# CLSFramework/gym-soccer-2d-env

Hardware: AMD Instinct MI355X
Metric: env-steps/sec at 65536 parallel reach_ball envs per MI355X (higher is better)
Workload: dtype f32

## Files before the change

gym-soccer-2d-env_amd/csrc/s2d_engine.hip:

```cpp
#include <hip/hip_runtime.h>

#include <cmath>
#include <cstdio>
#include <cstdlib>
#include <cstring>
#include <new>
#include <string>
#include <type_traits>

#include "s2d_device.h"

#include "s2d_actor_launch.h"
#include "s2d_kernels.h"

__global__ void s2d_tables_kernel(S2DHot p, const S2DRare* __restrict__ rp, S2DTables* __restrict__ t) {
  if (blockIdx.x == 0 && threadIdx.x == 0 && rp->tab_len > 0) tables_build(p, rp->recover_init, rp->tab_power, rp->tab_len, *t);
}
__global__ __launch_bounds__(kBlock) void s2d_init_kernel(S2DHot p, const S2DRare* __restrict__ rp,
                                                          float* __restrict__ S, int64_t stride, int64_t n) {
  int64_t i = (int64_t)blockIdx.x * kBlock + threadIdx.x;
  if (i >= n) return;
  S[F_STAMINA * stride + i] = p.stamina_max;
  S[F_RECOVERY * stride + i] = rp->recover_init;
  S[F_EFFORT * stride + i] = p.effort_init;
// ... 264 lines not shown
      sc_lut[k] = make_float2(sn, cs);
    }
    __syncthreads();
  }
  if (wave_first >= n) return;
  const bool active = i < n;
  int64_t rows = n - wave_first; if (rows > kWave) rows = kWave;
  const int valid = (int)rows * S2D_OBS_DIM;
  const bool use_k = uses_policy_step<MODE, NOISE>(kind);
  uint32_t* const kplane = reinterpret_cast<uint32_t*>(S + F_POLICY * stride);
  Env e;
  uint32_t gl = 0, gh = 0, k0 = 0;
  if (active) {
    env_load(e, S, stride, i);
    if (use_k) k0 = kplane[i];
    uint64_t gid = (((uint64_t)p.gid_hi << 32) | p.gid_lo) + (uint64_t)i;
    gl = (uint32_t)gid; gh = (uint32_t)(gid >> 32);
    asm volatile("" ::"v"(e.px), "v"(e.py), "v"(e.vx), "v"(e.vy), "v"(e.body), "v"(e.stamina), "v"(e.effort),
                 "v"(e.recovery), "v"(e.capacity), "v"(e.bx), "v"(e.by), "v"(e.bvx), "v"(e.bvy), "v"(e.prev_dist),
                 "v"(e.prev_angle), "v"(e.step_number), "v"(e.cycle), "v"(k0));
  }
  bool fast = false;
  if (tab_len > 0) {
    bool ok = true;
    if (active) {
      const int sn = e.step_number;
      ok = sn >= 0 && sn < tab_len;
      const int q = ok ? sn : 0;
      ok = ok && e.stamina == tb->stamina[q] && e.effort == tb->effort[q] && e.recovery == tb->recovery[q] &&
           e.capacity == tb->capacity[q] && e.body == rintf(e.body) && fabsf(e.body) <= 180.0f;
    }
    fast = __ballot(active && !ok) == 0ull;
  }
  ObsOut ob;
  float reward = 0.0f, dir = 0.0f; int done = 0, res = 0, cmd = 0;
  unsigned int cnt1 = 0, cnt2 = 0, cnt3 = 0;
  float* const term_row = o.terminal_obs + i * S2D_OBS_DIM;
  U4 quad{0, 0, 0, 0}, squad{0, 0, 0, 0};
  bool have_prep = false;
  uint32_t* const coop_scratch = reinterpret_cast<uint32_t*>(&lds[wv][0]);
  if (p.auto_reset) {
    prep_fill_coop<NK>(p, rp, prep[wv], lane, active ? reset_key(e) : 0u, gl, gh, active, coop_scratch);
    have_prep = active;
  }
  int n_missing = 0;
  int64_t row = 0;
  const bool lut = NOISE && MODE == S2D_MODE_DISCRETE && kind == S2D_ACT_RANDOM && p.n_actions <= kWave;
  if (lut && lane < p.n_actions) {
    int c0; float pw, d0;
    action_map<MODE>(p, Action4{(float)lane, 0.0f, 0.0f, 0.0f}, 0.0f, c0, pw, d0);
    const CmdPrep c = cmd_prepare(p, c0, pw, d0);
    act_lut[wv][lane] = make_float4(c.power, c.dir, c.dir_rate, d0);
  }
  for (int t = 0; t < n_steps; ++t, row += n) {
    res = 0;
    if (n_missing >= kRefillMin) {
      if (active && !have_prep) { prep_fill<NK>(p, rp, prep[wv], lane, e, gl, gh); have_prep = true; }
      n_missing = 0;
    }
    if (active) {
      const uint32_t k = k0 + (uint32_t)t;
      CmdPrep c;
      if (lut) {
        if (t == 0 || (k & 3u) == 0u) quad = policy_quad(p, gl, gh, k, S2D_ST_POLICY);
        const int a = (int)rnd_below(quad_word(quad, k), (uint32_t)p.n_actions);
        if (ro.action) static_cast<int32_t*>(ro.action)[row + i] = a;
        const float4 e4 = act_lut[wv][a];
        c = CmdPrep{e4.x, e4.y, e4.z}; dir = e4.w; cmd = S2D_CMD_DASH;
      } else {
        c = decide<MODE>(p, actions, kind, row + i, gl, gh, k, t == 0 || (k & 3u) == 0u, quad, squad, ro.action, cmd, dir);
      }
      if (fast) step_env<NK, true>(p, rp, e, gl, gh, k, cmd, c, ob, reward, done, res, term_row, &prep[wv], lane, have_prep, ep_lds, sc_lut);
      else step_env<NK, false>(p, rp, e, gl, gh, k, cmd, c, ob, reward, done, res, term_row, &prep[wv], lane, have_prep);
      if (ro.reward) ro.reward[row + i] = reward;
      if (ro.done) ro.done[row + i] = (uint8_t)done;
      if (ro.result) ro.result[row + i] = (uint8_t)res;
      cnt1 += res == S2D_RESULT_GOAL; cnt2 += res == S2D_RESULT_OUT; cnt3 += res == S2D_RESULT_TIMEOUT;
    }
    if (p.auto_reset) n_missing += __popcll(__ballot(active && done != 0));
    if (ro.obs) store_obs_tile(lds[wv], ob, lane, active, ro.obs + (row + wave_first) * S2D_OBS_DIM, valid);
  }
  if (active) {
    if (fast) {
      const int q = e.step_number;
      e.stamina = tb->stamina[q]; e.effort = tb->effort[q]; e.recovery = tb->recovery[q]; e.capacity = tb->capacity[q];
    }
    env_store(e, S, stride, i);
    if (use_k) kplane[i] = k0 + (uint32_t)n_steps;
    o.reward[i] = reward; o.done[i] = (uint8_t)done; o.result[i] = (uint8_t)res;
    o.action_dir[i] = dir; o.action_cmd[i] = (uint8_t)cmd;
  }
  store_obs_tile(lds[wv], ob, lane, active, o.obs + wave_first * S2D_OBS_DIM, valid);
  if (!active) { cnt1 = cnt2 = cnt3 = 0; }
#pragma unroll
  for (int off = 32; off > 0; off >>= 1) {
    cnt1 += __shfl_xor(cnt1, off); cnt2 += __shfl_xor(cnt2, off); cnt3 += __shfl_xor(cnt3, off);
  }
  unsigned long long* const srow = stats_row(o.stats, wave_first);
  stats_store(srow, lane, stats_load(srow, lane), wave_first == 0 ? (unsigned long long)n * (unsigned long long)n_steps : 0ull, cnt1, cnt2, cnt3);
}

#ifndef S2D_NPRIO_S
#define S2D_NPRIO_S 3
#endif
#ifndef S2D_NPRIO_A
#define S2D_NPRIO_A 2
#endif
#ifndef S2D_NPRIO_B
#define S2D_NPRIO_B 2
#endif
#ifndef S2D_NPRIO_P
#define S2D_NPRIO_P 1
#endif
#ifndef S2D_PRIO_S
#define S2D_PRIO_S 1
#endif
#ifndef S2D_PRIO_A
#define S2D_PRIO_A 2
#endif
#ifndef S2D_PRIO_B
#define S2D_PRIO_B 3
#endif

#ifdef S2D_STAMPS
#define WS_STAMP_DECL uint64_t st_busy = 0, st_t0 = __builtin_amdgcn_s_memtime(); const uint64_t st_begin = st_t0, st_rt0 = __builtin_amdgcn_s_memrealtime()
#define WS_BARRIER() do { st_busy += __builtin_amdgcn_s_memtime() - st_t0; __syncthreads(); st_t0 = __builtin_amdgcn_s_memtime(); } while (0)
#define WS_STAMP_STORE() do { if (lane == 0) { float* q_ = o.terminal_obs + (wave_first + 2 * role) * S2D_OBS_DIM; \
    q_[0] = (float)st_busy; q_[1] = (float)(__builtin_amdgcn_s_memtime() - st_begin); q_[2] = (float)(st_rt0 & 0xffffff); \
    q_[3] = (float)(__builtin_amdgcn_s_memrealtime() & 0xffffff); \
    q_[4] = __int_as_float((int)__builtin_amdgcn_s_getreg((31 << 11) | 4)); q_[5] = __int_as_float((int)__builtin_amdgcn_s_getreg((31 << 11) | 20)); } } while (0)
#else
#define WS_STAMP_DECL do {} while (0)
#define WS_BARRIER() __syncthreads()
#define WS_STAMP_STORE() do {} while (0)
#endif

template <int MODE, int NK, int REC = 0>
__global__ __launch_bounds__(kWsBlock, 4) void s2d_reach_rollout_ws_kernel(S2DHot p_sgpr, const S2DRare* __restrict__ rp,
                                                                        float* __restrict__ S, int64_t stride,
                                                                        int64_t n, int n_steps,
                                                                        const void* __restrict__ actions, int kind,
                                                                        RolloutOut ro, StepOut o) {
  constexpr bool NOISE = NK != S2D_NK_OFF;
  constexpr int kActWords = NOISE ? (int)WA_WORDS : (int)WA_NPM;
  __shared__ float act[3][kActWords][kWave];
  __shared__ float snap[2][WS_WORDS][kWave];
  __shared__ float slots[kSlots][SL_WORDS][kWave];
  __shared__ __attribute__((aligned(16))) float tile[2][kObsTile];
  __shared__ float4 act_lut[kWave];
  __shared__ float ep_lds[S2D_TAB_MAX];
  __shared__ float2 sc_lut[361];
  const int lane = threadIdx.x & (kWave - 1);
  const int role = __builtin_amdgcn_readfirstlane(threadIdx.x / kWave);
  const bool nt = REC == 2 || (REC == 0 && ro.nt != 0);
  const int64_t wave_first = (int64_t)blockIdx.x * kWave;
  const int64_t i = wave_first + lane;
  const bool active = i < n;
  int64_t rows = n - wave_first; rows = rows > kWave ? kWave : rows;
  const int valid = (int)rows * S2D_OBS_DIM;
  const int n_iter = n_steps + 3;

  if (role != 1 && p_sgpr.auto_reset) {
    const uint64_t gid = (((uint64_t)p_sgpr.gid_hi << 32) | p_sgpr.gid_lo) + (uint64_t)i;
    uint32_t ep0 = 0u;
    if (active) ep0 = reinterpret_cast<const uint32_t*>(S + F_EPISODE * stride)[i];
    const int k = role == 0 ? 0 : role - 1;
    slot_fill_coop<NK>(p_sgpr, rp, slots[k], lane, (uint32_t)gid, (uint32_t)(gid >> 32), ep0 + 1u + (uint32_t)k, active,
                          reinterpret_cast<uint32_t*>(&tile[0][0]) + role * kWave);
  }

  if (role == 0) {
    if constexpr (NOISE) __builtin_amdgcn_s_setprio(S2D_NPRIO_P);
    const S2DHot& p = p_sgpr;
    const bool use_k = uses_policy_step<MODE, NOISE>(kind);
    uint32_t* const kplane = reinterpret_cast<uint32_t*>(S + F_POLICY * stride);
    uint32_t gl = 0, gh = 0, k0 = 0;
    if (active) {
      if (use_k) k0 = kplane[i];
      uint64_t gid = (((uint64_t)p.gid_hi << 32) | p.gid_lo) + (uint64_t)i;
      gl = (uint32_t)gid; gh = (uint32_t)(gid >> 32);
    }
    U4 quad{0, 0, 0, 0}, squad{0, 0, 0, 0}, nblk{0, 0, 0, 0};
    float dir = 0.0f; int cmd = 0;
    int64_t row = 0;
    const bool lut = MODE == S2D_MODE_DISCRETE && kind == S2D_ACT_RANDOM && p.n_actions <= kWave;
    if (lut && lane < p.n_actions) {
      int c0; float pw, d0;
      action_map<MODE>(p, Action4{(float)lane, 0.0f, 0.0f, 0.0f}, 0.0f, c0, pw, d0);
      const CmdPrep c = cmd_prepare(p, c0, pw, d0);
      act_lut[lane] = make_float4(c.power, c.dir, c.dir_rate, d0);
    }
    __syncthreads();
    WS_STAMP_DECL;
    int wslot = 0;
    auto policy_step = [&](int t) {
      if (active) {
        const uint32_t k = k0 + (uint32_t)t;
        CmdPrep c;
        if (lut) {
          if (t == 0 || (k & 3u) == 0u) quad = policy_quad(p, gl, gh, k, S2D_ST_POLICY);
          const int a = (int)rnd_below(quad_word(quad, k), (uint32_t)p.n_actions);
          if (REC != 0 || ro.action) rec_store(static_cast<int32_t*>(ro.action) + row + i, (int32_t)a, nt);
          const float4 e4 = act_lut[a];
          c = CmdPrep{e4.x, e4.y, e4.z}; dir = e4.w; cmd = S2D_CMD_DASH;
        } else {
          c = decide<MODE>(p, actions, kind, row + i, gl, gh, k, t == 0 || (k & 3u) == 0u, quad, squad, ro.action, cmd, dir);
        }
        const int b = wslot;
        if (MODE == S2D_MODE_TURN4) act[b][WA_CMD][lane] = __int_as_float(cmd);
        act[b][WA_POWER][lane] = c.power;
        act[b][WA_DIR][lane] = c.dir; act[b][WA_RATE][lane] = c.dir_rate;
        if constexpr (NK == S2D_NK_SQUARE) {
          const NoiseIn nz = noise_prepare_square(p, gl, gh, k, S2D_ST_NOISE, cmd == S2D_CMD_TURN);
          act[b][WA_NPM][lane] = nz.pm; act[b][WA_NPS][lane] = nz.ps; act[b][WA_NPC][lane] = nz.pc;
          act[b][WA_NBM][lane] = nz.bm; act[b][WA_NBS][lane] = nz.bs; act[b][WA_NBC][lane] = nz.bc;
          if (MODE == S2D_MODE_TURN4) act[b][WA_NTU][lane] = nz.tu;
        } else if constexpr (NOISE) {
          const NoiseWords nw = noise_words(p, gl, gh, k, S2D_ST_NOISE, cmd == S2D_CMD_TURN, nblk, t == 0 || (k & 1u) == 0u);
          const float2 ps = sc_lut[noise_dir_index(nw.wp)], bs = sc_lut[noise_dir_index(nw.wb)];
          act[b][WA_NPM][lane] = noise_mag(nw.wp); act[b][WA_NPS][lane] = ps.x; act[b][WA_NPC][lane] = ps.y;
          act[b][WA_NBM][lane] = noise_mag(nw.wb); act[b][WA_NBS][lane] = bs.x; act[b][WA_NBC][lane] = bs.y;
          if (MODE == S2D_MODE_TURN4) act[b][WA_NTU][lane] = nw.tu;
        }
        row += n;
      }
      wslot = wslot == 2 ? 0 : wslot + 1;
    };
    for (int s = 0; s < n_iter; ++s) {
      if (s == 0 && n_steps > 0) policy_step(0);
      if (s + 1 < n_steps) policy_step(s + 1);
      WS_BARRIER();
    }
    WS_STAMP_STORE();
    if (active) {
      if (use_k) kplane[i] = k0 + (uint32_t)n_steps;
      o.action_dir[i] = dir; o.action_cmd[i] = (uint8_t)cmd;
    }
  } else if (role == 1) {
    if constexpr (NOISE) __builtin_amdgcn_s_setprio(S2D_NPRIO_S);
    else __builtin_amdgcn_s_setprio(S2D_PRIO_S);
    const S2DHot p = hot_in_vgprs(p_sgpr);
    Env e;
    uint32_t gl = 0, gh = 0;
    int nth = 0, j = 0;
    if (active) {
      env_load(e, S, stride, i);
      uint64_t gid = (((uint64_t)p.gid_hi << 32) | p.gid_lo) + (uint64_t)i;
      gl = (uint32_t)gid; gh = (uint32_t)(gid >> 32);
      asm volatile("" ::"v"(e.px), "v"(e.py), "v"(e.vx), "v"(e.vy), "v"(e.body), "v"(e.stamina), "v"(e.effort),
                   "v"(e.recovery), "v"(e.capacity), "v"(e.bx), "v"(e.by), "v"(e.bvx), "v"(e.bvy),
                   "v"(e.step_number), "v"(e.cycle), "v"(e.episode));
    }
    const S2DTables* const tb = tables_of(rp);
    const int tab_len = MODE != S2D_MODE_TURN4 ? rp->tab_len : 0;
    bool fast = false;
    if (tab_len > 0) {
      bool ok = true;
      if (active) {
        const int sn = e.step_number;
        ok = sn >= 0 && sn < tab_len;
        const int q = ok ? sn : 0;
        ok = ok && e.stamina == tb->stamina[q] && e.effort == tb->effort[q] && e.recovery == tb->recovery[q] &&
             e.capacity == tb->capacity[q] && e.body == rintf(e.body) && fabsf(e.body) <= 180.0f;
      }
      fast = __ballot(active && !ok) == 0ull;
      if (fast)
        for (int k = lane; k < tab_len; k += kWave) ep_lds[k] = tb->ep[k];
    }
    if (fast || NK == S2D_NK_LATTICE) {
      for (int k = lane; k <= 360; k += kWave) {
        float sn, cs;
        sincos_deg((float)(k - 180), sn, cs);
        sc_lut[k] = make_float2(sn, cs);
      }
    }
    const ResetStamina rst = reset_stamina(p, rp);
    __syncthreads();
    WS_STAMP_DECL;
    auto loop = [&](auto fast_tag) {
      constexpr bool FAST = decltype(fast_tag)::value;
      struct ActRegs { float cmd, power, dir, rate, npm, nps, npc, nbm, nbs, nbc, ntu; };
      ActRegs cur{}, nxt{};
      float ep_cur = 0.0f; float2 sc_cur = make_float2(0.0f, 0.0f);
      int rslot = 1;
      auto fetch = [&](int slot) {
        ActRegs r{};
        if (MODE == S2D_MODE_TURN4) r.cmd = act[slot][WA_CMD][lane];
        if (!FAST) r.power = act[slot][WA_POWER][lane];
        r.dir = act[slot][WA_DIR][lane]; r.rate = act[slot][WA_RATE][lane];
        if constexpr (NOISE) {
          r.npm = act[slot][WA_NPM][lane]; r.nps = act[slot][WA_NPS][lane]; r.npc = act[slot][WA_NPC][lane];
          r.nbm = act[slot][WA_NBM][lane]; r.nbs = act[slot][WA_NBS][lane]; r.nbc = act[slot][WA_NBC][lane];
          if (MODE == S2D_MODE_TURN4) r.ntu = act[slot][WA_NTU][lane];
        }
        return r;
      };
      auto lookups = [&]() {
        if constexpr (FAST) {
          ep_cur = ep_lds[e.step_number];
          sc_cur = sc_lut[(int)norm_deg(e.body + cur.dir) + 180];
        }
      };
      auto simulate_iteration = [&](int s, auto steady_tag) {
        constexpr bool STEADY = decltype(steady_tag)::value;
        if ((STEADY || (s >= 1 && s <= n_steps)) && active) {
          if (!STEADY && s == 1) { cur = fetch(0); lookups(); }
          const bool more = STEADY || s < n_steps;
          if (more) nxt = fetch(rslot);
          const int b = (s - 1) & 1;
          int cmd = S2D_CMD_DASH;
          if (MODE == S2D_MODE_TURN4) cmd = __float_as_int(cur.cmd);
          NoiseIn nz{0.0f, 0.0f, 0.0f, 0.0f, 0.0f, 0.0f, 0.0f};
          if constexpr (NOISE) {
            nz = NoiseIn{cur.npm, cur.nps, cur.npc, cur.nbm, cur.nbs, cur.nbc, 0.0f};
            if (MODE == S2D_MODE_TURN4) nz.tu = cur.ntu;
          }
          float d2;
          if constexpr (FAST) {
            e.step_number += 1;
            d2 = sim_cycle_dash_fast<NOISE>(p, rp, e, ep_cur, cur.rate, sc_cur.x, sc_cur.y, nz);
          } else {
            const CmdPrep c{cur.power, cur.dir, cur.rate};
            e.step_number += 1;
            d2 = sim_cycle<NOISE, true>(p, rp, e, cmd, c, nz);
          }
          int flags = judge_sq(p, e.px, e.py, d2, e.step_number);
          const bool took = flags && p.auto_reset;
          snap[b][WS_PX][lane] = e.px; snap[b][WS_PY][lane] = e.py; snap[b][WS_BODY][lane] = e.body;
          snap[b][WS_BX][lane] = e.bx; snap[b][WS_BY][lane] = e.by;
          snap[b][WS_BVX][lane] = e.bvx; snap[b][WS_BVY][lane] = e.bvy;
          snap[b][WS_FLAGS][lane] = __int_as_float(flags | (j << 8));
          if (took) {
            if (nth >= kSlots)
              slot_fill<NK>(p, rp, slots[j], lane, gl, gh, (uint32_t)e.episode + 1u);
            episode_begin(e, slot_take<kWave>(slots[j], lane, rst));
            nth += 1; j = (j + 1 == kSlots) ? 0 : j + 1;
          }
          if (more) { cur = nxt; lookups(); }
        }
        if (STEADY || (s >= 1 && s < n_steps)) rslot = rslot == 2 ? 0 : rslot + 1;
        WS_BARRIER();
      };
      int s = 0;
      for (; s < 2 && s < n_iter; ++s) simulate_iteration(s, std::false_type{});
      for (; s < n_steps; ++s) simulate_iteration(s, std::true_type{});
      for (; s < n_iter; ++s) simulate_iteration(s, std::false_type{});
    };
    if (fast) {
      loop(std::true_type{});
      if (active) {
        const int q = e.step_number;
        e.stamina = tb->stamina[q]; e.effort = tb->effort[q]; e.recovery = tb->recovery[q]; e.capacity = tb->capacity[q];
      }
    } else {
      loop(std::false_type{});
    }
    WS_STAMP_STORE();
    if (active) {
      S[F_PX * stride + i] = e.px; S[F_PY * stride + i] = e.py;
      S[F_VX * stride + i] = e.vx; S[F_VY * stride + i] = e.vy;
      S[F_BODY * stride + i] = e.body;
      S[F_STAMINA * stride + i] = e.stamina; S[F_EFFORT * stride + i] = e.effort;
      S[F_RECOVERY * stride + i] = e.recovery; S[F_CAPACITY * stride + i] = e.capacity;
      S[F_BX * stride + i] = e.bx; S[F_BY * stride + i] = e.by;
      S[F_BVX * stride + i] = e.bvx; S[F_BVY * stride + i] = e.bvy;
      S[F_STEP * stride + i] = __int_as_float(e.step_number);
      S[F_CYCLE * stride + i] = __int_as_float(e.cycle);
      S[F_EPISODE * stride + i] = __int_as_float(e.episode);
    }
  } else if (role == 2) {
    __builtin_amdgcn_s_setprio(NOISE ? S2D_NPRIO_A : S2D_PRIO_A);
    const S2DHot p = hot_in_vgprs(p_sgpr);
    const bool auto_reset = p_sgpr.auto_reset != 0;
    float prev_dist = 0.0f, prev_angle = 0.0f;
    if (active) {
      prev_dist = S[F_PREV_DIST * stride + i]; prev_angle = S[F_PREV_ANGLE * stride + i];
      asm volatile("" ::"v"(prev_dist), "v"(prev_angle));
    }
    float oa[S2D_OBS_DIM];
    float reward = 0.0f; int res = 0, done = 0;
    unsigned int cnt1 = 0, cnt2 = 0, cnt3 = 0;
    unsigned long long* const srow = stats_row(o.stats, wave_first);
    const unsigned long long sold = stats_load(srow, lane);
    float* const term_row = o.terminal_obs + i * S2D_OBS_DIM;
    int64_t row = 0;
    __syncthreads();
    WS_STAMP_DECL;
    auto agent_iteration = [&](int s, auto steady_tag) {
      constexpr bool STEADY = decltype(steady_tag)::value;
      if (STEADY || (s >= 2 && s < n_steps + 2)) {
        const int b = s & 1;
        res = 0;
        if (active) {
          float px = snap[b][WS_PX][lane], py = snap[b][WS_PY][lane], body = snap[b][WS_BODY][lane];
          float bx = snap[b][WS_BX][lane], by = snap[b][WS_BY][lane];
          const int fw = __float_as_int(snap[b][WS_FLAGS][lane]);
          const int flags = fw & 0xff;
          float dist = hypot2(bx - px, by - py);
          float rel = observe_player(p, px, py, body, bx, by, oa);
          reward = reward_of(prev_dist, prev_angle, dist, rel, flags, res);
          prev_dist = dist; prev_angle = rel;
          done = flags ? 1 : 0;
          if (flags && auto_reset) {
            const float (*sl)[kWave] = slots[fw >> 8];
#pragma unroll
            for (int k = 0; k < 4; ++k) term_row[k] = oa[k];
#pragma unroll
            for (int k = 0; k < 4; ++k) oa[k] = sl[SL_FIRST + k][lane];
            prev_dist = sl[SL_DIST][lane]; prev_angle = sl[SL_REL][lane];
          }
          if (REC != 0 || ro.reward) rec_store(ro.reward + row + i, reward, nt);
          if (REC != 0 || ro.done) rec_store(ro.done + row + i, (uint8_t)done, nt);
          if (REC != 0 || ro.result) rec_store(ro.result + row + i, (uint8_t)res, nt);
          cnt1 += res == S2D_RESULT_GOAL; cnt2 += res == S2D_RESULT_OUT; cnt3 += res == S2D_RESULT_TIMEOUT;
          if (REC != 0 || ro.obs) {
            float* t = &tile[b][lane * S2D_OBS_DIM];
            t[0] = oa[0]; t[1] = oa[1]; t[2] = oa[2]; t[3] = oa[3];
          }
        }
        row += n;
      }
      WS_BARRIER();
    };
    {
      int s = 0;
      for (; s < 3 && s < n_iter; ++s) agent_iteration(s, std::false_type{});
      for (; s < n_steps + 2; ++s) agent_iteration(s, std::true_type{});
      for (; s < n_iter; ++s) agent_iteration(s, std::false_type{});
    }
    WS_STAMP_STORE();
    if (active) {
      S[F_PREV_DIST * stride + i] = prev_dist; S[F_PREV_ANGLE * stride + i] = prev_angle;
      o.reward[i] = reward; o.done[i] = (uint8_t)done; o.result[i] = (uint8_t)res;
#pragma unroll
      for (int k = 0; k < 4; ++k) o.obs[i * S2D_OBS_DIM + k] = oa[k];
    }
    if (!active) { cnt1 = cnt2 = cnt3 = 0; }
#pragma unroll
    for (int off = 32; off > 0; off >>= 1) {
      cnt1 += __shfl_xor(cnt1, off); cnt2 += __shfl_xor(cnt2, off); cnt3 += __shfl_xor(cnt3, off);
    }
    stats_store(srow, lane, sold, wave_first == 0 ? (unsigned long long)n * (unsigned long long)n_steps : 0ull, cnt1, cnt2, cnt3);
  } else {
    if constexpr (NOISE) __builtin_amdgcn_s_setprio(S2D_NPRIO_B);
    else __builtin_amdgcn_s_setprio(S2D_PRIO_B);
    const S2DHot p = hot_in_vgprs(p_sgpr);
    const bool auto_reset = p_sgpr.auto_reset != 0;
    float ob6[S2D_OBS_DIM];
    float* const term_row = o.terminal_obs + i * S2D_OBS_DIM;
    const bool obs_all_vec = valid == kObsTile && ((n * S2D_OBS_DIM * 4) & 15) == 0 &&
                             (reinterpret_cast<uintptr_t>(ro.obs + wave_first * S2D_OBS_DIM) & 15u) == 0;
    __syncthreads();
    WS_STAMP_DECL;
    auto ball_iteration = [&](int s, auto steady_tag) {
      constexpr bool STEADY = decltype(steady_tag)::value;
      if ((STEADY || s >= 3) && (REC != 0 || ro.obs))
        tile_flush(tile[(s - 1) & 1], lane, ro.obs + ((int64_t)(s - 3) * n + wave_first) * S2D_OBS_DIM, valid, nt, obs_all_vec);
      if ((STEADY || (s >= 2 && s < n_steps + 2)) && active) {
        const int b = s & 1;
        float bx = snap[b][WS_BX][lane], by = snap[b][WS_BY][lane];
        float bvx = snap[b][WS_BVX][lane], bvy = snap[b][WS_BVY][lane];
        const int fw = __float_as_int(snap[b][WS_FLAGS][lane]);
        observe_ball(p, bx, by, bvx, bvy, ob6);
        if ((fw & 0xff) && auto_reset) {
          const float (*sl)[kWave] = slots[fw >> 8];
#pragma unroll
          for (int k = 4; k < S2D_OBS_DIM; ++k) term_row[k] = ob6[k];
#pragma unroll
          for (int k = 4; k < S2D_OBS_DIM; ++k) ob6[k] = sl[SL_FIRST + k][lane];
        }
        if (REC != 0 || ro.obs) {
          float* t = &tile[b][lane * S2D_OBS_DIM];
#pragma unroll
          for (int k = 4; k < S2D_OBS_DIM; ++k) t[k] = ob6[k];
        }
      }
      WS_BARRIER();
    };
    {
      int s = 0;
      for (; s < 3 && s < n_iter; ++s) ball_iteration(s, std::false_type{});
      for (; s < n_steps + 2; ++s) ball_iteration(s, std::true_type{});
      for (; s < n_iter; ++s) ball_iteration(s, std::false_type{});
    }
    WS_STAMP_STORE();
    if (active) {
#pragma unroll
      for (int k = 4; k < S2D_OBS_DIM; ++k) o.obs[i * S2D_OBS_DIM + k] = ob6[k];
    }
  }
}

__global__ __launch_bounds__(kBlock) void s2d_world_model_kernel(const float* __restrict__ S, int64_t stride,
                                                                 int64_t n, S2DWorldModel w) {
  int64_t i = (int64_t)blockIdx.x * kBlock + threadIdx.x;
  if (i >= n) return;
  float px = S[F_PX * stride + i], py = S[F_PY * stride + i], vx = S[F_VX * stride + i], vy = S[F_VY * stride + i];
  float bx = S[F_BX * stride + i], by = S[F_BY * stride + i], bvx = S[F_BVX * stride + i], bvy = S[F_BVY * stride + i];
  float dx = bx - px, dy = by - py;
  float dist = hypot2(dx, dy), ang = atan2_deg(dy, dx);
  if (w.ball_dist_from_self) w.ball_dist_from_self[i] = dist;
  if (w.ball_angle_from_self) w.ball_angle_from_self[i] = ang;
  if (w.ball_relative_x) w.ball_relative_x[i] = dx;
  if (w.ball_relative_y) w.ball_relative_y[i] = dy;
  if (w.ball_pos_dist) w.ball_pos_dist[i] = hypot2(bx, by);
  if (w.ball_pos_angle) w.ball_pos_angle[i] = atan2_deg(by, bx);
  if (w.ball_vel_dist) w.ball_vel_dist[i] = hypot2(bvx, bvy);
  if (w.ball_vel_angle) w.ball_vel_angle[i] = atan2_deg(bvy, bvx);
  if (w.self_pos_dist) w.self_pos_dist[i] = hypot2(px, py);
  if (w.self_pos_angle) w.self_pos_angle[i] = atan2_deg(py, px);
  if (w.self_vel_dist) w.self_vel_dist[i] = hypot2(vx, vy);
  if (w.self_vel_angle) w.self_vel_angle[i] = atan2_deg(vy, vx);
  if (w.self_dist_from_ball) w.self_dist_from_ball[i] = dist;
  if (w.self_angle_from_ball) w.self_angle_from_ball[i] = atan2_deg(-dy, -dx);
}

enum { SV_NONFINITE, SV_BODY, SV_STAMINA, SV_EFFORT_RECOVERY, SV_COUNTERS, SV_OBS, SV_WORDS = 8 };
__global__ __launch_bounds__(kBlock) void s2d_validate_kernel(S2DHot p, const float* __restrict__ S, int64_t stride, int64_t n,
                                                              const float* __restrict__ obs, unsigned int* __restrict__ out) {
  const int64_t i = (int64_t)blockIdx.x * kBlock + threadIdx.x;
  if (i >= n) return;
  Env e;
  env_load(e, S, stride, i);
  const float w[15] = {e.px, e.py, e.vx, e.vy, e.body, e.stamina, e.effort, e.recovery, e.capacity, e.bx, e.by, e.bvx, e.bvy,
                       e.prev_dist, e.prev_angle};
  bool finite = true;
#pragma unroll
  for (int k = 0; k < 15; ++k) finite = finite && isfinite(w[k]);
  bool obs_ok = true;
#pragma unroll
  for (int k = 0; k < S2D_OBS_DIM; ++k) obs_ok = obs_ok && isfinite(obs[i * S2D_OBS_DIM + k]);
  if (!finite) atomicAdd(&out[SV_NONFINITE], 1u);
  if (!(fabsf(e.body) <= 180.0f) || !(fabsf(e.prev_angle) <= 180.0f)) atomicAdd(&out[SV_BODY], 1u);
  if (!(e.stamina >= 0.0f && e.stamina <= p.stamina_max) || !(e.capacity >= 0.0f || p.stamina_capacity < 0.0f)) atomicAdd(&out[SV_STAMINA], 1u);
  if (!(e.effort >= p.effort_min && e.effort <= p.effort_init) || !(e.recovery >= p.recover_min && e.recovery <= p.recover_init))
    atomicAdd(&out[SV_EFFORT_RECOVERY], 1u);
  if (e.step_number < 0 || e.episode < 0 || !(e.prev_dist >= 0.0f)) atomicAdd(&out[SV_COUNTERS], 1u);
  if (!obs_ok) atomicAdd(&out[SV_OBS], 1u);
}

__global__ void s2d_debug_eval_kernel(int op, const float* __restrict__ in, float* __restrict__ out, int64_t n) {
  int64_t i = (int64_t)blockIdx.x * blockDim.x + threadIdx.x;
  if (op == 9) {
    __shared__ uint32_t scratch[256];
    const uint32_t* u = reinterpret_cast<const uint32_t*>(in) + 4 * i;
    S2DHot p{}; p.seed_lo = u[2]; p.seed_hi = 0x5EEDu; p.half_l = 52.5f; p.half_w = 34.0f;
    S2DRare r{}; r.change_ball_position = 1; r.change_ball_velocity = 1; r.travel_factor = __uint_as_float(u[3]);
    const int lane = threadIdx.x & 63;
    const ResetSample a = reset_sample_coop(p, r, (uint32_t)i, 7u, u[0], u[1] != 0u, lane, scratch + (threadIdx.x & ~63u));
    const ResetSample b = reset_sample(p, r, (uint32_t)i, 7u, u[0]);
    float* q = out + 14 * i;
    q[0] = a.px; q[1] = a.py; q[2] = a.body; q[3] = a.bx; q[4] = a.by; q[5] = a.bvx; q[6] = a.bvy;
    q[7] = b.px; q[8] = b.py; q[9] = b.body; q[10] = b.bx; q[11] = b.by; q[12] = b.bvx; q[13] = b.bvy;
    return;
  }
  if (i >= n) return;
  switch (op) {
    case 10: {
      const uint32_t* u = reinterpret_cast<const uint32_t*>(in) + 4 * i;
      S2DHot p{}; p.seed_lo = u[3]; p.seed_hi = 0u;
      const NoiseIn nz = noise_prepare(p, u[0], u[1], u[2], S2D_ST_NOISE, false);
      float* q = out + 6 * i;
      q[0] = nz.pm; q[1] = nz.ps; q[2] = nz.pc; q[3] = nz.bm; q[4] = nz.bs; q[5] = nz.bc;
      break;
    }
    case 11:
    case 12: {
      const uint32_t* u = reinterpret_cast<const uint32_t*>(in) + 4 * i;
      S2DHot p{}; p.seed_lo = u[3]; p.seed_hi = 0u;
      const NoiseIn nz = noise_prepare_square(p, u[0], u[1], u[2], op == 11 ? S2D_ST_NOISE : S2D_ST_NOISE_RESET, false);
      float* q = out + 4 * i;
      q[0] = nz.pc; q[1] = nz.ps; q[2] = nz.bc; q[3] = nz.bs;
      break;
    }
    case 13: out[i] = tanh_spec(in[i]); break;
    case 14: out[i] = log_spec(in[i]); break;
    case 15: {
      const uint32_t* u = reinterpret_cast<const uint32_t*>(in) + 4 * i;
      S2DHot p{}; p.seed_lo = u[3]; p.seed_hi = 0u;
      const U4 w = s2d_draw(p, u[0], u[1], u[2], S2D_ST_POLICY, 3);
      float* q = out + 4 * i;
      box_muller(w.x, w.y, q[0], q[1]);
      box_muller(w.z, w.w, q[2], q[3]);
      break;
    }
    case 0: { float s, c; sincos_deg(in[i], s, c); out[2 * i] = s; out[2 * i + 1] = c; break; }
    case 1: out[i] = atan2_deg(in[2 * i], in[2 * i + 1]); break;
    case 2: out[i] = exp_spec(in[i]); break;
    case 3: out[i] = norm_deg_any(in[i]); break;
    case 4: {
      const uint32_t* u = reinterpret_cast<const uint32_t*>(in) + 6 * i;
      U4 r = philox4x32_10(u[0], u[1], u[2], u[3], u[4], u[5]);
      uint32_t* q = reinterpret_cast<uint32_t*>(out) + 4 * i;
      q[0] = r.x; q[1] = r.y; q[2] = r.z; q[3] = r.w;
      break;
    }
    case 5: out[i] = hypot2(in[2 * i], in[2 * i + 1]); break;
    case 6: {
      const float* r = in + 9 * i;
      S2DHot p{}; p.inv_half_l = r[7]; p.inv_half_w = r[8];
      ObsOut ob;
      observe(p, r[4], r[5], r[6], r[0], r[1], r[2], r[3], ob);
      for (int k = 0; k < S2D_OBS_DIM; ++k) out[S2D_OBS_DIM * i + k] = ob.o[k];
      break;
    }
    case 7: {
      const float* r = in + 8 * i;
      S2DHot p{}; p.act_scale = r[6];
      const Action4 a{r[0], r[1], r[2], r[3]};
      int cmd = 0; float power = 0.0f, dir = 0.0f;
// ... 765 lines not shown
```

gym-soccer-2d-env_amd/csrc/s2d_kernels.h:

```cpp
#pragma once
#include <hip/hip_runtime.h>

#include <type_traits>

#include "s2d_device.h"
#include "s2d_net.h"

#define S2D_API extern "C" __attribute__((visibility("default")))

#ifndef S2D_BLOCK
#define S2D_BLOCK 256
#endif
static constexpr int kBlock = S2D_BLOCK;
static constexpr int kWavesPerBlock = kBlock / kWave;
static constexpr int kObsTile = kWave * S2D_OBS_DIM;
static constexpr int64_t kWsMaxEnvs = 524288;

struct StepOut {
  float* obs;
  float* reward;
  uint8_t* done;
  uint8_t* result;
  float* terminal_obs;
  float* action_dir;
  uint8_t* action_cmd;
  unsigned long long* stats;
  float* prep;
};

enum { PS_PX, PS_PY, PS_BODY, PS_BX, PS_BY, PS_BVX, PS_BVY, PS_WORDS };
S2D_DEV uint32_t* prep_tags(float* prep, int64_t stride) { return reinterpret_cast<uint32_t*>(prep + 2 * PS_WORDS * stride); }
static constexpr uint32_t kPrepTagMask = 0x3fffffffu;
S2D_DEV uint32_t prep_tag_of(uint32_t episode, const NextEpisode& q) {
  return (episode & kPrepTagMask) | ((uint32_t)__float_as_int(q.vx) & 0x80000000u) | (((uint32_t)__float_as_int(q.vy) & 0x80000000u) >> 1);
}

S2D_DEV void wave_lds_fence() {
  __builtin_amdgcn_fence(__ATOMIC_RELEASE, "wavefront");
  __builtin_amdgcn_wave_barrier();
  __builtin_amdgcn_fence(__ATOMIC_ACQUIRE, "wavefront");
}

S2D_DEV void tile_write(float* tile, const ObsOut& ob, int lane, bool active) {
  if (active) {
#pragma unroll
    for (int k = 0; k < S2D_OBS_DIM; ++k) tile[lane * S2D_OBS_DIM + k] = ob.o[k];
  }
}
typedef float v4f32_t __attribute__((ext_vector_type(4)));
S2D_DEV void rec_store16(float4* p, const float4& v, bool nt) {
  if (nt) {
    const v4f32_t w = {v.x, v.y, v.z, v.w};
    asm volatile("global_store_dwordx4 %0, %1, off nt" ::"v"(p), "v"(w) : "memory");
  } else {
    *p = v;
  }
}
template <typename T>
S2D_DEV void rec_store(T* p, T v, bool nt) {
  if (nt) __builtin_nontemporal_store(v, p); else *p = v;
}
S2D_DEV void tile_flush(const float* tile, int lane, float* __restrict__ dst, int valid, bool nt = false, bool all_vec = false) {
  const bool vec = all_vec || ((valid == kObsTile) && ((reinterpret_cast<uintptr_t>(dst) & 15u) == 0));
  if (vec) {
    const float4* t4 = reinterpret_cast<const float4*>(tile);
    float4* d4 = reinterpret_cast<float4*>(dst);
    rec_store16(d4 + lane, t4[lane], nt);
    rec_store16(d4 + kWave + lane, t4[kWave + lane], nt);
    if (lane < 32) rec_store16(d4 + 2 * kWave + lane, t4[2 * kWave + lane], nt);
  } else {
#pragma unroll
    for (int j = 0; j < S2D_OBS_DIM; ++j) {
      int idx = j * kWave + lane;
      if (idx < valid) dst[idx] = tile[idx];
    }
  }
}
S2D_DEV void store_obs_tile(float* tile, const ObsOut& ob, int lane, bool active, float* __restrict__ dst,
                            int valid) {
  tile_write(tile, ob, lane, active);
  wave_lds_fence();
  tile_flush(tile, lane, dst, valid);
  wave_lds_fence();
}

S2D_DEV unsigned long long* stats_row(unsigned long long* stats, int64_t wave_first) { return stats + (wave_first / kWave) * 8; }
S2D_DEV unsigned long long stats_load(const unsigned long long* row, int lane) { return lane < 4 ? row[lane] : 0ull; }
S2D_DEV void stats_store(unsigned long long* row, int lane, unsigned long long old, unsigned long long steps, unsigned int goal,
                         unsigned int out, unsigned int timeout) {
  const unsigned long long add = lane == 0 ? steps : lane == 1 ? goal : lane == 2 ? out : timeout;
  if (lane < 4 && add != 0ull) row[lane] = old + add;
}
S2D_DEV unsigned int wave_count(bool pred) { return (unsigned int)__popcll(__ballot(pred)); }

template <int MODE>
S2D_DEV Action4 load_action(const void* __restrict__ actions, int kind, int64_t idx) {
  Action4 a{0.0f, 0.0f, 0.0f, 0.0f};
  if (MODE == S2D_MODE_DISCRETE) {
    a.a0 = (kind == S2D_ACT_DISCRETE_I64) ? (float)static_cast<const long long*>(actions)[idx]
                                          : (float)static_cast<const int32_t*>(actions)[idx];
  } else if (MODE == S2D_MODE_CONT1) {
    a.a0 = static_cast<const float*>(actions)[idx];
  } else {
    float4 v = static_cast<const float4*>(actions)[idx];
    a.a0 = v.x; a.a1 = v.y; a.a2 = v.z; a.a3 = v.w;
  }
  return a;
}
template <int MODE>
S2D_DEV Action4 random_action(const S2DHot& p, uint32_t gid_lo, uint32_t gid_hi, uint32_t k, U4& quad, bool refresh) {
  Action4 a{0.0f, 0.0f, 0.0f, 0.0f};
  if (MODE == S2D_MODE_TURN4) {
    U4 w = s2d_draw(p, gid_lo, gid_hi, k, S2D_ST_POLICY, 1);
    a.a0 = rnd_u01(w.x) * 2.0f - 1.0f; a.a1 = rnd_u01(w.y) * 2.0f - 1.0f;
    a.a2 = rnd_u01(w.z) * 2.0f - 1.0f; a.a3 = rnd_u01(w.w) * 2.0f - 1.0f;
  } else {
    if (refresh) quad = policy_quad(p, gid_lo, gid_hi, k, S2D_ST_POLICY);
    uint32_t w = quad_word(quad, k);
    if (MODE == S2D_MODE_DISCRETE) a.a0 = (float)rnd_below(w, (uint32_t)p.n_actions);
    else a.a0 = rnd_u01(w) * 2.0f - 1.0f;
  }
  return a;
}
template <int MODE, bool NOISE>
S2D_DEV bool uses_policy_step(int kind) { return kind == S2D_ACT_RANDOM || MODE == S2D_MODE_TURN4 || NOISE; }

template <int MODE>
S2D_DEV void store_rollout_action(void* __restrict__ dst, int64_t idx, const Action4& a) {
  if (MODE == S2D_MODE_DISCRETE) static_cast<int32_t*>(dst)[idx] = (int32_t)a.a0;
  else if (MODE == S2D_MODE_CONT1) static_cast<float*>(dst)[idx] = a.a0;
  else static_cast<float4*>(dst)[idx] = make_float4(a.a0, a.a1, a.a2, a.a3);
}

template <int MODE>
S2D_DEV CmdPrep decide(const S2DHot& p, const void* __restrict__ actions, int kind, int64_t idx, uint32_t gid_lo,
                       uint32_t gid_hi, uint32_t k, bool refresh, U4& quad, U4& squad, void* __restrict__ action_out,
                       int& cmd, float& dir) {
  if (kind == S2D_ACT_COMMAND) {
    const float4 v = static_cast<const float4*>(actions)[idx];
    cmd = command_code(v.x); dir = v.z;
    return cmd_prepare(p, cmd, v.y, v.z);
  }
  Action4 a = (kind == S2D_ACT_RANDOM) ? random_action<MODE>(p, gid_lo, gid_hi, k, quad, refresh)
                                       : load_action<MODE>(actions, kind, idx);
  if (action_out) store_rollout_action<MODE>(action_out, idx, a);
  float u = 0.0f;
  if (MODE == S2D_MODE_TURN4) {
    if (refresh) squad = policy_quad(p, gid_lo, gid_hi, k, S2D_ST_SELECT);
    u = rnd_u01(quad_word(squad, k));
  }
  float power;
  action_map<MODE>(p, a, u, cmd, power, dir);
  return cmd_prepare(p, cmd, power, dir);
}

template <int MODE>
S2D_DEV CmdPrep decode_action(const S2DHot& p, const Action4& a, uint32_t gl, uint32_t gh, uint32_t k, bool refresh, U4& squad,
                              int& cmd, float& dir) {
  float u = 0.0f;
  if (MODE == S2D_MODE_TURN4) {
    if (refresh) squad = policy_quad(p, gl, gh, k, S2D_ST_SELECT);
    u = rnd_u01(quad_word(squad, k));
  }
  float power;
  action_map<MODE>(p, a, u, cmd, power, dir);
  return cmd_prepare(p, cmd, power, dir);
}

struct PrepTile { float v[13 + S2D_OBS_DIM + 2][kWave]; };
#ifndef S2D_REFILL_MIN
#define S2D_REFILL_MIN 8
#endif
static constexpr int kRefillMin = S2D_REFILL_MIN;

template <int NK>
S2D_DEV void prep_fill(const S2DHot& p, const S2DRare* __restrict__ rp, PrepTile& t, int lane, const Env& e,
                       uint32_t gid_lo, uint32_t gid_hi) {
  const S2DRare r = *rp;
  const NextEpisode q = episode_prepare<NK>(p, rp, r, gid_lo, gid_hi, reset_key(e));
  t.v[0][lane] = q.px; t.v[1][lane] = q.py; t.v[2][lane] = q.vx; t.v[3][lane] = q.vy; t.v[4][lane] = q.body;
  t.v[5][lane] = q.stamina; t.v[6][lane] = q.effort; t.v[7][lane] = q.recovery; t.v[8][lane] = q.capacity;
  t.v[9][lane] = q.bx; t.v[10][lane] = q.by; t.v[11][lane] = q.bvx; t.v[12][lane] = q.bvy;
  const FirstObs f = first_obs(p, q);
#pragma unroll
  for (int k = 0; k < S2D_OBS_DIM; ++k) t.v[13 + k][lane] = f.o[k];
  t.v[13 + S2D_OBS_DIM][lane] = f.dist; t.v[14 + S2D_OBS_DIM][lane] = f.rel;
}
template <int NK>
S2D_DEV void prep_fill_coop(const S2DHot& p, const S2DRare* __restrict__ rp, PrepTile& t, int lane, uint32_t key,
                            uint32_t gid_lo, uint32_t gid_hi, bool need, uint32_t* scratch) {
  const S2DRare r = *rp;
  const NextEpisode q = episode_prepare_coop<NK>(p, rp, r, gid_lo, gid_hi, key, need, lane, scratch);
  const FirstObs f = first_obs(p, q);
  if (need) {
    t.v[0][lane] = q.px; t.v[1][lane] = q.py; t.v[2][lane] = q.vx; t.v[3][lane] = q.vy; t.v[4][lane] = q.body;
    t.v[5][lane] = q.stamina; t.v[6][lane] = q.effort; t.v[7][lane] = q.recovery; t.v[8][lane] = q.capacity;
    t.v[9][lane] = q.bx; t.v[10][lane] = q.by; t.v[11][lane] = q.bvx; t.v[12][lane] = q.bvy;
#pragma unroll
    for (int k = 0; k < S2D_OBS_DIM; ++k) t.v[13 + k][lane] = f.o[k];
    t.v[13 + S2D_OBS_DIM][lane] = f.dist; t.v[14 + S2D_OBS_DIM][lane] = f.rel;
  }
}
S2D_DEV NextEpisode prep_take_episode(const PrepTile& t, int lane) {
  return NextEpisode{t.v[0][lane], t.v[1][lane], t.v[2][lane], t.v[3][lane], t.v[4][lane], t.v[5][lane], t.v[6][lane],
                     t.v[7][lane], t.v[8][lane], t.v[9][lane], t.v[10][lane], t.v[11][lane], t.v[12][lane]};
}

S2D_DEV const S2DTables* tables_of(const S2DRare* rp) {
  return reinterpret_cast<const S2DTables*>(reinterpret_cast<const char*>(rp) + 256);
}

template <int NK, bool FAST = false>
S2D_DEV void step_env(const S2DHot& p, const S2DRare* __restrict__ rp, Env& e, uint32_t gid_lo, uint32_t gid_hi,
                      uint32_t k, int cmd, const CmdPrep& c, ObsOut& ob, float& reward, int& done, int& result,
// ... 117 lines not shown
```

Measured before the change: 104.7 billion.

## Remap blocks across XCDs and limit nontemporal stores to observation output

Adds an XCD-aware block-to-env mapping, so that consecutive env ranges go to blocks dispatched on the same XCD (eight-way round-robin deal). This is meant to improve L2 locality of the state and output writes. Nontemporal stores are now used only for observation tiles; action, reward, done and result stores go through the normal cached path. The scalar nontemporal stores are replaced with inline-asm global_store with the nt bit. The remap assumes eight XCDs and round-robin dispatch, and changes which workgroup handles which envs.

```diff
diff --git a/gym-soccer-2d-env_amd/csrc/s2d_block_map.h b/gym-soccer-2d-env_amd/csrc/s2d_block_map.h
--- /dev/null
+++ b/gym-soccer-2d-env_amd/csrc/s2d_block_map.h
@@ -0,0 +1,15 @@
+#pragma once
+
+#if defined(__HIPCC__)
+#define S2D_HOST_DEVICE __host__ __device__
+#else
+#define S2D_HOST_DEVICE
+#endif
+
+static constexpr unsigned kXcdDeal = 8;
+
+S2D_HOST_DEVICE inline unsigned ws_env_block(unsigned block, unsigned n_blocks) {
+  const unsigned x = block % kXcdDeal, j = block / kXcdDeal;
+  const unsigned q = n_blocks / kXcdDeal, r = n_blocks % kXcdDeal;
+  return x * q + (x < r ? x : r) + j;
+}
diff --git a/gym-soccer-2d-env_amd/csrc/s2d_engine.hip b/gym-soccer-2d-env_amd/csrc/s2d_engine.hip
--- a/gym-soccer-2d-env_amd/csrc/s2d_engine.hip
+++ b/gym-soccer-2d-env_amd/csrc/s2d_engine.hip
@@ -440,8 +440,12 @@
   __shared__ float2 sc_lut[361];
   const int lane = threadIdx.x & (kWave - 1);
   const int role = __builtin_amdgcn_readfirstlane(threadIdx.x / kWave);
-  const bool nt = REC == 2 || (REC == 0 && ro.nt != 0);
-  const int64_t wave_first = (int64_t)blockIdx.x * kWave;
+  constexpr int kStreamNt = REC_NT_OBS;
+  const bool stream = REC == 2 || (REC == 0 && ro.nt != 0);
+  const bool nt_action = stream && (kStreamNt & REC_NT_ACTION), nt_reward = stream && (kStreamNt & REC_NT_REWARD);
+  const bool nt_labels = stream && (kStreamNt & REC_NT_LABELS), nt_obs = stream && (kStreamNt & REC_NT_OBS);
+  const unsigned n_blocks = (unsigned)((n + kWave - 1) / kWave);
+  const int64_t wave_first = (int64_t)ws_env_block(blockIdx.x, n_blocks) * kWave;
   const int64_t i = wave_first + lane;
   const bool active = i < n;
   int64_t rows = n - wave_first; rows = rows > kWave ? kWave : rows;
@@ -488,7 +492,7 @@
         if (lut) {
           if (t == 0 || (k & 3u) == 0u) quad = policy_quad(p, gl, gh, k, S2D_ST_POLICY);
           const int a = (int)rnd_below(quad_word(quad, k), (uint32_t)p.n_actions);
-          if (REC != 0 || ro.action) rec_store(static_cast<int32_t*>(ro.action) + row + i, (int32_t)a, nt);
+          if (REC != 0 || ro.action) rec_store(static_cast<int32_t*>(ro.action) + row + i, (int32_t)a, nt_action);
           const float4 e4 = act_lut[a];
           c = CmdPrep{e4.x, e4.y, e4.z}; dir = e4.w; cmd = S2D_CMD_DASH;
         } else {
@@ -697,9 +701,9 @@
             for (int k = 0; k < 4; ++k) oa[k] = sl[SL_FIRST + k][lane];
             prev_dist = sl[SL_DIST][lane]; prev_angle = sl[SL_REL][lane];
           }
-          if (REC != 0 || ro.reward) rec_store(ro.reward + row + i, reward, nt);
-          if (REC != 0 || ro.done) rec_store(ro.done + row + i, (uint8_t)done, nt);
-          if (REC != 0 || ro.result) rec_store(ro.result + row + i, (uint8_t)res, nt);
+          if (REC != 0 || ro.reward) rec_store(ro.reward + row + i, reward, nt_reward);
+          if (REC != 0 || ro.done) rec_store(ro.done + row + i, (uint8_t)done, nt_labels);
+          if (REC != 0 || ro.result) rec_store(ro.result + row + i, (uint8_t)res, nt_labels);
           cnt1 += res == S2D_RESULT_GOAL; cnt2 += res == S2D_RESULT_OUT; cnt3 += res == S2D_RESULT_TIMEOUT;
           if (REC != 0 || ro.obs) {
             float* t = &tile[b][lane * S2D_OBS_DIM];
@@ -743,7 +747,7 @@
     auto ball_iteration = [&](int s, auto steady_tag) {
       constexpr bool STEADY = decltype(steady_tag)::value;
       if ((STEADY || s >= 3) && (REC != 0 || ro.obs))
-        tile_flush(tile[(s - 1) & 1], lane, ro.obs + ((int64_t)(s - 3) * n + wave_first) * S2D_OBS_DIM, valid, nt, obs_all_vec);
+        tile_flush(tile[(s - 1) & 1], lane, ro.obs + ((int64_t)(s - 3) * n + wave_first) * S2D_OBS_DIM, valid, nt_obs, obs_all_vec);
       if ((STEADY || (s >= 2 && s < n_steps + 2)) && active) {
         const int b = s & 1;
         float bx = snap[b][WS_BX][lane], by = snap[b][WS_BY][lane];
diff --git a/gym-soccer-2d-env_amd/csrc/s2d_kernels.h b/gym-soccer-2d-env_amd/csrc/s2d_kernels.h
--- a/gym-soccer-2d-env_amd/csrc/s2d_kernels.h
+++ b/gym-soccer-2d-env_amd/csrc/s2d_kernels.h
@@ -3,6 +3,7 @@
 
 #include <type_traits>
 
+#include "s2d_block_map.h"
 #include "s2d_device.h"
 #include "s2d_net.h"
 
@@ -56,10 +57,19 @@
     *p = v;
   }
 }
-template <typename T>
-S2D_DEV void rec_store(T* p, T v, bool nt) {
-  if (nt) __builtin_nontemporal_store(v, p); else *p = v;
-}
+S2D_DEV void rec_store(float* p, float v, bool nt) {
+  if (nt) asm volatile("global_store_dword %0, %1, off nt" ::"v"(p), "v"(v) : "memory");
+  else *p = v;
+}
+S2D_DEV void rec_store(int32_t* p, int32_t v, bool nt) {
+  if (nt) asm volatile("global_store_dword %0, %1, off nt" ::"v"(p), "v"(v) : "memory");
+  else *p = v;
+}
+S2D_DEV void rec_store(uint8_t* p, uint8_t v, bool nt) {
+  if (nt) asm volatile("global_store_byte %0, %1, off nt" ::"v"(p), "v"((uint32_t)v) : "memory");
+  else *p = v;
+}
+enum { REC_NT_ACTION = 1, REC_NT_REWARD = 2, REC_NT_LABELS = 4, REC_NT_OBS = 8, REC_NT_ALL = 15 };
 S2D_DEV void tile_flush(const float* tile, int lane, float* __restrict__ dst, int valid, bool nt = false, bool all_vec = false) {
   const bool vec = all_vec || ((valid == kObsTile) && ((reinterpret_cast<uintptr_t>(dst) & 15u) == 0));
   if (vec) {
```

Measured after the change: 106.6 billion, median of 6. 1.8% higher.
